# KatiaJDL/CenterPoly

Measured on AMD Instinct MI355X. Metric: inference img/s @2048x1024 DLA-34 (1 GPU), higher is better.
Workload: dtype f32 I/O; split-bf16 x3 contraction (a*b ~ ah*bh + ah*bl + al*bh on bf16 MFMA, ~2^-16 per product) in the convolutions, the heads and DCNv2; f32 accumulate; 1 GPU; BASELINE config 2: DLA-34 + DCNv2, 1x3x1024x2048 synthetic, 16-vertex cartesian head, K=128, forward + sigmoid + NMS/top-k/decode; parallelism=single

## Files before the change

centerpoly_amd/_C.py:

```python
import ctypes
import os
from ctypes import POINTER, Structure, c_char_p, c_float, c_int32, c_int64, c_size_t, c_void_p

import torch

_HERE = os.path.dirname(os.path.abspath(__file__))
LIB_PATH = os.path.join(_HERE, "csrc", "libcenterpoly_hip.so")

CP_OK = 0
REP = {"cartesian": 0, "polar": 1, "polar_fixed": 2}
HEATMAP_UMICH, HEATMAP_ELLIPSE = 0, 1
L1_PLAIN, L1_POLAR, L1_POLAR_FIXED, L1_RELU20, L1_SMOOTH = 0, 1, 2, 3, 4
DCN_BWD_EXACT_F32, DCN_BWD_NARROW_TILES = 1, 2
DCN_CONTRACTION = {"f32": 0, "bf16x3": 1, "bf16x3_region": 3}


class DcnShape(Structure):
    _fields_ = [(n, c_int32) for n in ("B", "Cin", "H", "W", "Cout", "kh", "kw", "stride", "pad",
                                       "dil", "deformable_groups")]


class TargetShape(Structure):
    _fields_ = [(n, c_int32) for n in ("B", "max_objs", "nbr_points", "num_classes", "out_h", "out_w",
                                       "rep", "no_reorder_flip")]
# ... 13 lines not shown
    pass


_lib = None

ABI_VERSION = 3
_P = c_void_p
_SIGNATURES = {
    "cp_abi_version": (c_int32, []),
    "cp_strerror": (c_char_p, [c_int32]),
    "cp_build_arch": (c_char_p, []),
    "cp_dcn_v2_forward_workspace_bytes": (c_size_t, [POINTER(DcnShape)]),
    "cp_dcn_v2_forward_kernel": (c_int32, [POINTER(DcnShape), c_int32]),
    "cp_dcn_v2_forward": (c_int32, [POINTER(DcnShape), _P, _P, c_int64, _P, c_int64, c_int32, _P, _P,
                                    _P, _P, c_int32, c_int32, _P, _P, c_size_t, _P]),
    "cp_dcn_v2_forward_fused_supported": (c_int32, [POINTER(DcnShape)]),
    "cp_dcn_v2_forward_fused_workspace_bytes": (c_size_t, [POINTER(DcnShape)]),
    "cp_dcn_v2_forward_fused": (c_int32, [POINTER(DcnShape), _P, _P, _P, _P, _P, _P, _P, c_int32, c_int32, _P, _P, _P,
                                          c_size_t, _P]),
    "cp_dcn_v2_backward_workspace_bytes": (c_size_t, [POINTER(DcnShape)]),
    "cp_dcn_v2_backward": (c_int32, [POINTER(DcnShape), _P, _P, c_int64, _P, c_int64, c_int32, _P, _P,
                                     _P, _P, c_int64, _P, c_int64, _P, _P, c_int32, _P, c_size_t, _P]),
    "cp_upsample2x_add": (c_int32, [_P, _P, _P] + [c_int32] * 4 + [_P]),
    "cp_depthwise_up_forward": (c_int32, [_P, _P, _P, _P] + [c_int32] * 5 + [_P]),
    "cp_depthwise_up_backward": (c_int32, [_P, _P, _P, _P, _P] + [c_int32] * 5 + [_P]),
    "cp_bn_workspace_bytes": (c_size_t, [c_int32, c_int32, c_int64]),
    "cp_bn_act_forward_train": (c_int32, [_P] * 9 + [c_float, c_float, c_int32, c_int32, c_int32, c_int64,
                                                    _P, c_size_t, _P]),
    "cp_bn_act_backward": (c_int32, [_P] * 7 + [c_int32] + [_P] * 4 + [c_int32, c_int32, c_int64, _P,
                                                                       c_size_t, _P]),
# ... 217 lines not shown
```

centerpoly_amd/csrc/dcn_fwd.hip:

```cpp
#include "cp_common.h"
#include "dcn_internal.h"
#include <stdlib.h>

namespace {

constexpr int BM = 64;
constexpr int TAPS = 9;
#ifndef CP_DCN_LDPAD
#define CP_DCN_LDPAD 2
#endif
constexpr int LDPAD = CP_DCN_LDPAD;
typedef unsigned u32x2 __attribute__((ext_vector_type(2)));
typedef float f32x2 __attribute__((ext_vector_type(2)));

struct DcnFwdArgs {
  const float* x;
  const float* offset;
  const float* mask;
  const float* weight;
  const float* bias;
  const float* ep_scale;
  const float* ep_shift;
  float* out;
  float* partial;
// ... 397 lines not shown
        *reinterpret_cast<f32x4*>(dst) = f32x4{v[0], v[1], v[2], v[3]};
      } else {
#pragma unroll
        for (int r = 0; r < 4; ++r)
          if (pp + r < HWo) dst[r] = v[r];
      }
    }
  }
}

__global__ __launch_bounds__(256) void dcn_splitk_reduce_kernel(DcnFwdArgs a, long long n_per_b) {
  const long long total = (long long)a.B * n_per_b;
  const int HWo = a.Ho * a.Wo;
  for (long long i = (long long)blockIdx.x * 256 + threadIdx.x; i < total;
       i += (long long)gridDim.x * 256) {
    float v = 0.f;
    for (int sidx = 0; sidx < a.splitk; ++sidx) v += a.partial[(long long)sidx * total + i];
    const int co = (int)((i % n_per_b) / HWo);
    float sc = 1.f, sh = 0.f;
    if (a.ep_scale) sc = a.ep_scale[co];
    if (a.ep_shift) sh = a.ep_shift[co];
    else if (a.bias) sh = a.bias[co];
    v = v * sc + sh;
    if (a.relu) v = fmaxf(v, 0.f);
    a.out[i] = v;
  }
}

struct Plan {
  int bn, splitk, c_per_split;
};

Plan make_plan(int B, int Cin, int Cout, int HWo) {
  const long long tiles_m = (long long)((HWo + BM - 1) / BM) * B;
  Plan p;
  p.bn = Cout > 64 ? 128 : 64;
  const long long blocks = tiles_m * ((Cout + p.bn - 1) / p.bn);
  p.splitk = 1;
  const int kc = 4;
  if (blocks < 384) {
    int s = (int)((512 + blocks - 1) / blocks);
// ... 115 lines not shown
  const bool prepared = contraction == CP_DCN_BF16X3_PREPARED || contraction == CP_DCN_BF16X3_REGION_PREPARED;
  const bool bf = contraction == CP_DCN_BF16X3 || contraction == CP_DCN_BF16X3_PREPARED || force_region;
  if (force_region && !cp_dcn_region_supported(s)) return CP_EUNSUPPORTED;
  if (bf && cp_dcn_region_supported(s) && (force_region || region_pays(s))) {
    if (!workspace || workspace_bytes < cp_dcn_v2_forward_workspace_bytes(s)) return CP_EWORKSPACE;
    hipStream_t st = (hipStream_t)stream;
    if (!prepared) {
      const int rc = cp_dcn_region_prepare(s, weight, workspace, st);
      if (rc != CP_OK) return rc;
    }
    const int ks = region_ksplit(s);
    float* partial = ks > 1 ? (float*)((char*)workspace + wpb) : nullptr;
    const int rc = cp_dcn_region_forward(s, x, offset, offset_bstride, mask, mask_bstride, mask_is_logit, workspace, bias,
                                         ep_scale, ep_shift, relu, out, nullptr, nullptr, nullptr, partial, ks, st);
    if (rc != CP_OK || ks <= 1) return rc;
    DcnFwdArgs ra;
    ra.partial = partial; ra.out = out; ra.bias = bias; ra.ep_scale = ep_scale; ra.ep_shift = ep_shift; ra.relu = relu;
    ra.B = s->B; ra.Ho = Ho; ra.Wo = Wo; ra.Cout = s->Cout; ra.splitk = ks;
    const long long n_per_b = (long long)s->Cout * Ho * Wo;
    long long nb = ((long long)s->B * n_per_b + 255) / 256;
    if (nb > 4096) nb = 4096;
    hipLaunchKernelGGL(dcn_splitk_reduce_kernel, dim3((unsigned)nb), dim3(256), 0, st, ra, n_per_b);
    return cp_launch_status();
  }
  if (p.splitk > 1 || bf) {
    if (!workspace || workspace_bytes < cp_dcn_v2_forward_workspace_bytes(s)) return CP_EWORKSPACE;
  }
  DcnFwdArgs a;
  a.x = x; a.offset = offset; a.mask = mask; a.weight = weight; a.bias = bias;
  a.ep_scale = ep_scale; a.ep_shift = ep_shift; a.out = out; a.partial = (float*)((char*)workspace + (workspace ? wpb : 0));
  a.offset_bstride = offset_bstride; a.mask_bstride = mask_bstride;
  a.B = s->B; a.Cin = s->Cin; a.H = s->H; a.W = s->W; a.Cout = s->Cout; a.Ho = Ho; a.Wo = Wo;
  a.stride = s->stride; a.pad = s->pad; a.dil = s->dil;
  a.mask_is_logit = mask_is_logit; a.relu = relu;
  a.splitk = p.splitk; a.c_per_split = p.c_per_split;
#ifdef CP_ABLATE
  {
// ... 4 lines not shown
  hipStream_t st = (hipStream_t)stream;
  CP_CHECK_ARG(contraction == CP_DCN_F32 || bf);
  if ((unsigned long long)s->Cout * s->Cin * 9ull * 4ull >= 0xE0000000ull) return CP_EUNSUPPORTED;
  if (bf && p.bn <= 128 && (p.c_per_split % 8) == 0) {
    if (!prepared) {
      const int nchunk = (s->Cin + 7) / 8;
      const int total = (int)(wperm_bytes_gather(s->Cin, s->Cout) / 16);
      hipLaunchKernelGGL(dcn_fwd_wperm_kernel, dim3((total + 255) / 256), dim3(256), 0, st, weight, (bf16x8*)workspace,
                         s->Cout, s->Cin, nchunk, total);
    }
    if (p.bn == 64) return launch_bf16x3<64, 2>(a, workspace, st);
    return launch_bf16x3<128, 2>(a, workspace, st);
  }
  if (p.bn == 64) return launch_pipe<64, 3>(a, st);
  return launch_pipe<128, 2>(a, st);
}

static size_t fused_region_bytes(const cp_dcn_shape* s) { return cp_align_up(cp_dcn_region_wperm_bytes(s), 256); }

extern "C" int cp_dcn_v2_forward_fused_supported(const cp_dcn_shape* s) {
  return s && s->B > 0 && s->Cout > 0 && s->Cout <= 64 && s->Cin <= 64 && cp_dcn_region_supported(s) && region_pays(s) &&
                 region_ksplit(s) == 1
             ? 1
             : 0;
}

extern "C" size_t cp_dcn_v2_forward_fused_workspace_bytes(const cp_dcn_shape* s) {
  if (!cp_dcn_v2_forward_fused_supported(s)) return 0;
  return fused_region_bytes(s) + cp_align_up(cp_dcn_region_om_wperm_bytes(s), 256);
}
// ... 20 lines not shown
```

centerpoly_amd/csrc/dcn_internal.h:

```cpp
#pragma once
#include "cp_common.h"

static inline int out_extent(int in, int pad, int dil, int stride) {
  return (in + 2 * pad - (dil * 2 + 1)) / stride + 1;
}

bool cp_dcn_region_supported(const cp_dcn_shape* s);
size_t cp_dcn_region_wperm_bytes(const cp_dcn_shape* s);
int cp_dcn_region_prepare(const cp_dcn_shape* s, const float* weight, void* wp, hipStream_t st);
size_t cp_dcn_region_om_wperm_bytes(const cp_dcn_shape* s);
int cp_dcn_region_prepare_om(const cp_dcn_shape* s, const float* om_weight, void* wp, hipStream_t st);
int cp_dcn_region_ksplit(const cp_dcn_shape* s);
int cp_dcn_region_forward(const cp_dcn_shape* s, const float* x, const float* offset, int64_t offset_bstride,
                          const float* mask, int64_t mask_bstride, int32_t mask_is_logit, const void* wp,
                          const float* bias, const float* ep_scale, const float* ep_shift, int32_t relu, float* out,
                          const void* om_wp, const float* om_bias, float* om_out, float* partial, int ksplit,
                          hipStream_t st);

bool cp_dcn_bwd_data2_supported(const cp_dcn_shape* s);
size_t cp_dcn_bwd_data2_workspace_bytes(const cp_dcn_shape* s);
int cp_dcn_bwd_data2(const cp_dcn_shape* s, const float* x, const float* offset, int64_t offset_bstride,
                     const float* mask, int64_t mask_bstride, int32_t mask_is_logit, const float* weight,
                     const float* grad_out, float* grad_x, float* grad_offset, int64_t grad_offset_bstride,
                     float* grad_mask, int64_t grad_mask_bstride, int32_t flags, void* workspace, size_t workspace_bytes,
// ... 7 lines not shown
```

centerpoly_amd/csrc/upsample.hip:

```cpp
#include "cp_common.h"

namespace {

typedef float f32x2 __attribute__((ext_vector_type(2)));

template <int F>
__global__ __launch_bounds__(256) void dw_up_kernel(const float* __restrict__ x,
                                                    const float* __restrict__ w,
                                                    const float* __restrict__ skip,
                                                    float* __restrict__ out, int C, int H, int W) {
  constexpr int KS = 2 * F, PAD = F / 2;
  const int Ho = H * F, Wo = W * F;
  const int bc = blockIdx.z;
  const int c = bc % C;
  const int oy = blockIdx.y;
  const int ox0 = (blockIdx.x * 256 + threadIdx.x) * 4;
  if (ox0 >= Wo) return;
  const float* wc = w + (long long)c * KS * KS;
  const float* xc = x + (long long)bc * H * W;
  const int ky0 = (oy + PAD) % F;
  const int iy0 = (oy + PAD - ky0) / F;
  float v[4] = {0.f, 0.f, 0.f, 0.f};
#pragma unroll
  for (int r = 0; r < 2; ++r) {
// ... 14 lines not shown
  }
  const long long o = ((long long)bc * Ho + oy) * Wo + ox0;
  if (skip) {
    if (ox0 + 3 < Wo) {
      const f32x4 s = *reinterpret_cast<const f32x4*>(skip + o);
      v[0] += s[0]; v[1] += s[1]; v[2] += s[2]; v[3] += s[3];
    } else {
      for (int q = 0; q < 4 && ox0 + q < Wo; ++q) v[q] += skip[o + q];
    }
  }
  if (ox0 + 3 < Wo) *reinterpret_cast<f32x4*>(out + o) = f32x4{v[0], v[1], v[2], v[3]};
  else
    for (int q = 0; q < 4 && ox0 + q < Wo; ++q) out[o + q] = v[q];
}

__global__ __launch_bounds__(256) void dw_up2_kernel(const float* __restrict__ x, const float* __restrict__ w,
                                                     const float* __restrict__ skip, float* __restrict__ out, int C, int H,
                                                     int W) {
  const int W2 = W >> 1;
  const int bc = blockIdx.y;
  const int idx = blockIdx.x * 256 + threadIdx.x;
  if (idx >= H * W2) return;
  const int i = idx / W2, j = idx - i * W2;
  const float* wc = w + (long long)(bc % C) * 16;
  float wk[4][4];
#pragma unroll
  for (int a = 0; a < 4; ++a)
#pragma unroll
    for (int b = 0; b < 4; ++b) wk[a][b] = wc[a * 4 + b];
  const float* xc = x + (long long)bc * H * W;
  float in[3][4];
#pragma unroll
  for (int r = 0; r < 3; ++r) {
    const int iy = i - 1 + r;
    const bool rok = iy >= 0 && iy < H;
    const float* row = xc + (long long)(rok ? iy : i) * W + 2 * j;
    const f32x2 mid = *reinterpret_cast<const f32x2*>(row);
    const float lft = j > 0 ? row[-1] : 0.f, rgt = 2 * j + 2 < W ? row[2] : 0.f;
    in[r][0] = rok ? lft : 0.f;
    in[r][1] = rok ? mid[0] : 0.f;
    in[r][2] = rok ? mid[1] : 0.f;
    in[r][3] = rok ? rgt : 0.f;
  }
  const int Wo = 2 * W;
  const long long o = ((long long)bc * 2 * H + 2 * i) * Wo + 4 * j;
#pragma unroll
  for (int e = 0; e < 2; ++e) {
    const float* hi = in[1 + e];
    const float* lo = in[e];
    const float* wa = wk[1 - e];
    const float* wb = wk[3 - e];
    f32x4 v;
    v[0] = hi[1] * wa[1] + hi[0] * wa[3] + lo[1] * wb[1] + lo[0] * wb[3];
    v[1] = hi[2] * wa[0] + hi[1] * wa[2] + lo[2] * wb[0] + lo[1] * wb[2];
    v[2] = hi[2] * wa[1] + hi[1] * wa[3] + lo[2] * wb[1] + lo[1] * wb[3];
    v[3] = hi[3] * wa[0] + hi[2] * wa[2] + lo[3] * wb[0] + lo[2] * wb[2];
    if (skip) {
      const f32x4 sk = *reinterpret_cast<const f32x4*>(skip + o + (long long)e * Wo);
      v[0] += sk[0]; v[1] += sk[1]; v[2] += sk[2]; v[3] += sk[3];
    }
    *reinterpret_cast<f32x4*>(out + o + (long long)e * Wo) = v;
  }
}

}

extern "C" int cp_depthwise_up_forward(const float* x, const float* weight, const float* skip,
                                       float* out, int32_t B, int32_t C, int32_t H, int32_t W,
                                       int32_t f, void* stream) {
  CP_CHECK_ARG(x && weight && out && B > 0 && C > 0 && H > 0 && W > 0);
  if (f != 2 && f != 4 && f != 8) return CP_EUNSUPPORTED;
  if ((W * f) % 4 != 0 || (long long)B * C > 65535 || (long long)H * f > 65535) return CP_EUNSUPPORTED;
  const int Wo = W * f, Ho = H * f;
  dim3 grid((Wo / 4 + 255) / 256, Ho, B * C);
  hipStream_t st = (hipStream_t)stream;
  if (f == 2 && (W & 1) == 0 && (long long)H * (W / 2) < (1ll << 31) - 256) {
    const dim3 g2((unsigned)(((long long)H * (W / 2) + 255) / 256), B * C);
    hipLaunchKernelGGL(dw_up2_kernel, g2, dim3(256), 0, st, x, weight, skip, out, C, H, W);
  } else if (f == 2) hipLaunchKernelGGL(dw_up_kernel<2>, grid, dim3(256), 0, st, x, weight, skip, out, C, H, W);
  else if (f == 4) hipLaunchKernelGGL(dw_up_kernel<4>, grid, dim3(256), 0, st, x, weight, skip, out, C, H, W);
  else hipLaunchKernelGGL(dw_up_kernel<8>, grid, dim3(256), 0, st, x, weight, skip, out, C, H, W);
  return cp_launch_status();
}

namespace {
__global__ __launch_bounds__(256) void bias_act_kernel(float* __restrict__ y,
                                                       const float* __restrict__ bias,
                                                       const float* __restrict__ res, int C,
                                                       long long HW, int relu) {
  const int bc = blockIdx.y;
  const float bv = bias ? bias[bc % C] : 0.f;
  float* yp = y + (long long)bc * HW;
  const float* rp = res ? res + (long long)bc * HW : nullptr;
  const long long n4 = HW >> 2;
  for (long long i = (long long)blockIdx.x * 256 + threadIdx.x; i < n4; i += (long long)gridDim.x * 256) {
    f32x4 v = reinterpret_cast<f32x4*>(yp)[i];
// ... 379 lines not shown
```

centerpoly_amd/models/networks/DCNv2/dcn_v2.py:

```python
import math
import os

import torch
import torch.nn.functional as F
import torch.nn as nn
from torch.nn.modules.utils import _pair

from .... import _C
from ..conv3x3 import conv_bias_act, conv_infer, conv_raw
from ..prepared import prepared


def _shape(x, weight, stride, pad, dil, dg):
    s = _C.DcnShape()
    s.B, s.Cin, s.H, s.W = x.shape
    s.Cout, _, s.kh, s.kw = weight.shape
    s.stride, s.pad, s.dil, s.deformable_groups = stride, pad, dil, dg
    return s


_AUTO = {}


def auto_contraction(s):
# ... 25 lines not shown
        if not built:
            mode += 1
    elif nws:
        ws = _C.workspace(nws, x.device)
    timer = _C.kernel_timer
    end = timer.start(("dcn_fwd", s.Cin, s.Cout, Ho, Wo, s.B)) if timer is not None else None
    rc = L.cp_dcn_v2_forward(s, _C.ptr(x), _C.ptr(om), bs, mask_ptr, bs, 1, _C.ptr(weight),
                             _C.ptr(bias), _C.ptr(ep_scale), _C.ptr(ep_shift), 1 if relu else 0,
                             mode, _C.ptr(out), _C.ptr(ws), nws, _C.stream())
    if end is not None:
        end.record()
    _C.check(rc, "cp_dcn_v2_forward")
    return out


def dcn_v2_module_forward(x, om_weight, om_bias, weight, bias, ep_scale=None, ep_shift=None, relu=False, owner=None,
                          want_om=False):
    L = _C.lib()
    s = _shape(x, weight, 1, 1, 1, 1)
    if tuple(weight.shape[2:]) != (3, 3) or tuple(om_weight.shape) != (27, s.Cin, 3, 3) \
            or not L.cp_dcn_v2_forward_fused_supported(s):
        return None
    nws = L.cp_dcn_v2_forward_fused_workspace_bytes(s)
    ws, built = (_C.workspace(nws, x.device), True) if owner is None else \
        prepared(owner, "dcn_fused", (weight, om_weight), lambda: _C.workspace(nws, x.device), tuple(x.shape))
    out = torch.empty((s.B, s.Cout, s.H, s.W), dtype=torch.float32, device=x.device)
    om = torch.empty((s.B, 27, s.H, s.W), dtype=torch.float32, device=x.device) if want_om else None
    timer = _C.kernel_timer
    end = timer.start(("dcn_fwd", s.Cin, s.Cout, s.H, s.W, s.B)) if timer is not None else None
    rc = L.cp_dcn_v2_forward_fused(s, _C.ptr(x), _C.ptr(om_weight), _C.ptr(om_bias), _C.ptr(weight), _C.ptr(bias),
# ... 174 lines not shown
    def forward_fused(self, x, ep_scale, ep_shift, relu=True):
        cm = self.conv_offset_mask
        con = getattr(self, "contraction", None) or DCN.infer_contraction
        if DCN.fuse_offset_conv and con in ("auto", "bf16x3") and x.is_cuda and x.dtype == torch.float32 \
                and self.stride == 1 and self.padding == 1 and self.dilation == 1 and self.deformable_groups == 1:
            r = dcn_v2_module_forward(x.contiguous(), cm.weight, cm.bias, self.weight, None, ep_scale, ep_shift, relu,
                                      owner=self)
            if r is not None:
                return r[0]
        om = conv_infer([x], cm, cm.weight, cm.bias, conv=cm)
        if om is None:
            om = cm(x)
        return dcn_v2_forward_raw(x.contiguous(), om.contiguous(), self.weight, None, self.stride,
                                  self.padding, self.dilation, self.deformable_groups, ep_scale,
                                  ep_shift, relu, getattr(self, "contraction", None) or DCN.infer_contraction, owner=self)
```

centerpoly_amd/models/networks/pose_dla_dcn.py:

```python
import math
import os

import numpy as np
import torch
import torch.nn.functional as F
from torch import nn

from ... import _C
from .DCNv2.dcn_v2 import DCN, conv_bias
from . import conv3x3
from .conv3x3 import conv_infer, conv_raw
from .prepared import prepared, release_inference

HEADS_FUSED = True
CONV_DIRECT_WGRAD = True

BN_MOMENTUM = 0.1


def _bn(c):
    return nn.BatchNorm2d(c, momentum=BN_MOMENTUM)



# ... 358 lines not shown
                              root_dim=root_dim + out_channels, **kw)
        self.downsample = nn.MaxPool2d(stride, stride=stride) if stride > 1 else None
        self.project = None
        if in_channels != out_channels:
            self.project = nn.Sequential(nn.Conv2d(in_channels, out_channels, 1, 1, bias=False),
                                         _bn(out_channels))
        self.project_is_dead = levels > 1 and self.project is not None
        if self.project_is_dead:
            for prm in self.project.parameters():
                prm.requires_grad_(False)

    def fold(self):
        self._folded = _fold_conv_bn(self.project[0], self.project[1]) if self.project is not None \
            else None

    def forward(self, x, residual=None, children=None):
        children = [] if children is None else children
        bottom = x if self.downsample is None else downsample2(self.downsample, x)
        if self.project is None:
            residual = bottom
        elif self.project_is_dead:
            residual = None
            if self.training:
                with torch.no_grad():
                    if bottom.is_cuda:
                        bn_act(self.project[1], conv_train(self.project[0], bottom), relu=False)
                    else:
                        self.project(bottom)
        elif _use_folded(self):
            residual = _conv_folded(bottom, self.project[0], self._folded)
        else:
            residual = bn_act(self.project[1], conv_train(self.project[0], bottom), relu=False)
        if self.level_root:
            children.append(bottom)
        x1 = self.tree1(x, residual)
        if self.levels == 1:
            return self.root(self.tree2(x1), x1, *children)
        children.append(x1)
        return self.tree2(x1, children=children)


class DLA(nn.Module):
    def __init__(self, levels, channels, num_classes=1000, block=BasicBlock, residual_root=False,
                 linear_root=False):
        super().__init__()
        self.channels, self.num_classes = channels, num_classes
        c = channels
        self.base_layer = nn.Sequential(nn.Conv2d(3, c[0], 7, 1, 3, bias=False), _bn(c[0]),
                                        nn.ReLU(inplace=True))
        self.level0 = self._conv_level(c[0], c[0], levels[0])
# ... 90 lines not shown
        return scale.contiguous(), shift.contiguous()

    def fold(self):
        with torch.no_grad():
            self._folded = self.folded_affine()

    def forward(self, x):
        if not self.training and not torch.is_grad_enabled():
            scale, shift = self._folded if getattr(self, "_folded", None) is not None \
                else self.folded_affine()
            return self.conv.forward_fused(x, scale, shift, relu=True)
        if self.training:
            return bn_act(self.actf[0], self.conv(x), relu=True)
        return self.actf(self.conv(x))


def depthwise_up_add(x, up, skip):
    L = _C.lib()
    B, C, H, W = x.shape
    f = up.stride[0]
    out = torch.empty((B, C, H * f, W * f), dtype=torch.float32, device=x.device)
    x, skip = x.contiguous(), skip.contiguous()
    rc = L.cp_depthwise_up_forward(_C.ptr(x), _C.ptr(up.weight), _C.ptr(skip), _C.ptr(out), B, C, H,
                                   W, f, _C.stream())
    _C.check(rc, "cp_depthwise_up_forward")
    return out


class _DepthwiseUpAdd(torch.autograd.Function):

# ... 13 lines not shown
    @staticmethod
    def backward(ctx, go):
        x, weight = ctx.saved_tensors
        L = _C.lib()
        go = go.contiguous()
        B, C, H, W = x.shape
        gx = torch.empty_like(x)
        gw = _C.zeros(weight.shape, weight.device)
        rc = L.cp_depthwise_up_backward(_C.ptr(x), _C.ptr(weight), _C.ptr(go), _C.ptr(gx), _C.ptr(gw),
                                        B, C, H, W, ctx.f, _C.stream())
        _C.check(rc, "cp_depthwise_up_backward")
        return gx, gw, go, None


class IDAUp(nn.Module):
    def __init__(self, o, channels, up_f):
        super().__init__()
        for i in range(1, len(channels)):
            f = int(up_f[i])
            up = nn.ConvTranspose2d(o, o, f * 2, stride=f, padding=f // 2, output_padding=0,
                                    groups=o, bias=False)
            fill_up_weights(up)
            setattr(self, "proj_%d" % i, DeformConv(channels[i], o))
            setattr(self, "up_%d" % i, up)
            setattr(self, "node_%d" % i, DeformConv(o, o))

    def forward(self, layers, startp, endp):
        fused = not self.training and not torch.is_grad_enabled()
        for i in range(startp + 1, endp):
            k = i - startp
            up, proj = getattr(self, "up_%d" % k), getattr(self, "proj_%d" % k)
            aligned = layers[i].is_cuda and (layers[i].shape[3] * up.stride[0]) % 4 == 0
            if fused and aligned and up.stride[0] in (2, 4, 8):
                summed = depthwise_up_add(proj(layers[i]), up, layers[i - 1])
            elif not fused and aligned and up.stride[0] in (2, 4):
                summed = _DepthwiseUpAdd.apply(proj(layers[i]), up.weight, layers[i - 1], up.stride[0])
            else:
                summed = up(proj(layers[i])) + layers[i - 1]
            layers[i] = getattr(self, "node_%d" % k)(summed)


class DLAUp(nn.Module):
    def __init__(self, startp, channels, scales, in_channels=None):
        super().__init__()
        self.startp = startp
        in_channels = list(channels) if in_channels is None else in_channels
        self.channels = channels
        channels = list(channels)
        scales = np.array(scales, dtype=int)
# ... 188 lines not shown
```

include/centerpoly_hip.h:

```cpp
#ifndef CENTERPOLY_HIP_H
#define CENTERPOLY_HIP_H

#include <stddef.h>
#include <stdint.h>

#ifdef __cplusplus
extern "C" {
#endif

#define CP_ABI_VERSION 3

enum {
  CP_OK = 0,
  CP_EINVAL = -1,
  CP_EUNSUPPORTED = -2,
  CP_EWORKSPACE = -3,
  CP_EHIP = -4
};

enum { CP_REP_CARTESIAN = 0, CP_REP_POLAR = 1, CP_REP_POLAR_FIXED = 2 };

enum {
  CP_DCN_F32 = 0,
  CP_DCN_BF16X3 = 1,
// ... 16 lines not shown

typedef struct cp_dcn_shape {
  int32_t B, Cin, H, W, Cout;
  int32_t kh, kw, stride, pad, dil;
  int32_t deformable_groups;
} cp_dcn_shape;

size_t cp_dcn_v2_forward_workspace_bytes(const cp_dcn_shape* s);
int cp_dcn_v2_forward_kernel(const cp_dcn_shape* s, int32_t contraction);
int cp_dcn_v2_forward(const cp_dcn_shape* s, const float* x, const float* offset,
                      int64_t offset_bstride, const float* mask, int64_t mask_bstride,
                      int32_t mask_is_logit, const float* weight, const float* bias,
                      const float* ep_scale, const float* ep_shift, int32_t relu,
                      int32_t contraction, float* out, void* workspace, size_t workspace_bytes,
                      void* stream);

int cp_dcn_v2_forward_fused_supported(const cp_dcn_shape* s);
size_t cp_dcn_v2_forward_fused_workspace_bytes(const cp_dcn_shape* s);
int cp_dcn_v2_forward_fused(const cp_dcn_shape* s, const float* x, const float* om_weight, const float* om_bias,
                            const float* weight, const float* bias, const float* ep_scale, const float* ep_shift,
                            int32_t relu, int32_t prepared, float* om_out, float* out, void* workspace,
                            size_t workspace_bytes, void* stream);

enum {
  CP_DCN_BWD_EXACT_F32 = 1,
  CP_DCN_BWD_NARROW_TILES = 2
};
size_t cp_dcn_v2_backward_workspace_bytes(const cp_dcn_shape* s);
int cp_dcn_v2_backward(const cp_dcn_shape* s, const float* x, const float* offset,
                       int64_t offset_bstride, const float* mask, int64_t mask_bstride,
                       int32_t mask_is_logit, const float* weight, const float* grad_out,
                       float* grad_x, float* grad_offset, int64_t grad_offset_bstride,
                       float* grad_mask, int64_t grad_mask_bstride, float* grad_weight,
                       float* grad_bias, int32_t flags, void* workspace, size_t workspace_bytes, void* stream);

int cp_depthwise_up_forward(const float* x, const float* weight, const float* skip, float* out,
                            int32_t B, int32_t C, int32_t H, int32_t W, int32_t f, void* stream);
int cp_depthwise_up_backward(const float* x, const float* weight, const float* grad_out,
                             float* grad_x, float* grad_weight, int32_t B, int32_t C, int32_t H,
                             int32_t W, int32_t f, void* stream);

int cp_maxpool2x2_forward(const float* x, float* out, int32_t B, int32_t C, int32_t H, int32_t W, void* stream);
int cp_maxpool2x2_backward(const float* x, const float* grad_out, float* grad_in, int32_t B, int32_t C, int32_t H,
                           int32_t W, void* stream);

int cp_upsample2x_add(const float* a, const float* low, float* out, int32_t B, int32_t C, int32_t H, int32_t W,
                      void* stream);

int cp_bias_act_inplace(float* y, const float* bias, const float* residual, int32_t B, int32_t C,
                        int64_t HW, int32_t relu, void* stream);
int cp_bias_relu_backward(const float* y, const float* grad_out, float* grad_in, float* grad_bias,
                          int32_t B, int32_t C, int64_t HW, void* stream);
// ... 259 lines not shown
```

Measured before the change: 358.1 img/s.

## Fold DCN split-K reduction into depthwise upsample-add and share Tree pooling

In IDAUp, the DCN projection now leaves its split-K partial slices in the workspace. A new tiled depthwise-upsample kernel sums those slices, applies the folded BN affine and ReLU in shared memory, then performs the 2x transposed depthwise upsample plus skip add. This removes the separate split-K reduce kernel and one full round trip of the projection output through memory. It also adds a dedicated 4x upsample kernel, an unrolled slice-summing helper, and reuse of the downsampled tensor between a Tree and its tree1 child at inference, so the same maxpool is not computed twice.

```diff
diff --git a/centerpoly_amd/_C.py b/centerpoly_amd/_C.py
--- a/centerpoly_amd/_C.py
+++ b/centerpoly_amd/_C.py
@@ -51,6 +51,11 @@
     "cp_dcn_v2_forward_kernel": (c_int32, [POINTER(DcnShape), c_int32]),
     "cp_dcn_v2_forward": (c_int32, [POINTER(DcnShape), _P, _P, c_int64, _P, c_int64, c_int32, _P, _P,
                                     _P, _P, c_int32, c_int32, _P, _P, c_size_t, _P]),
+    "cp_dcn_v2_forward_slices_count": (c_int32, [POINTER(DcnShape), c_int32]),
+    "cp_dcn_v2_forward_slices": (c_int32, [POINTER(DcnShape), _P, _P, c_int64, _P, c_int64, c_int32, _P, c_int32, _P,
+                                           c_size_t, POINTER(c_size_t), _P]),
+    "cp_dcn_splitk_reduce": (c_int32, [_P, c_int32, _P, _P, c_int32, _P, c_int32, c_int32, c_int64, _P]),
+    "cp_depthwise_up_forward_slices": (c_int32, [_P, c_int32, c_int64, _P, _P, c_int32, _P, _P, _P] + [c_int32] * 5 + [_P]),
     "cp_dcn_v2_forward_fused_supported": (c_int32, [POINTER(DcnShape)]),
     "cp_dcn_v2_forward_fused_workspace_bytes": (c_size_t, [POINTER(DcnShape)]),
     "cp_dcn_v2_forward_fused": (c_int32, [POINTER(DcnShape), _P, _P, _P, _P, _P, _P, _P, c_int32, c_int32, _P, _P, _P,
diff --git a/centerpoly_amd/csrc/dcn_fwd.hip b/centerpoly_amd/csrc/dcn_fwd.hip
--- a/centerpoly_amd/csrc/dcn_fwd.hip
+++ b/centerpoly_amd/csrc/dcn_fwd.hip
@@ -435,17 +435,27 @@
   const int HWo = a.Ho * a.Wo;
   for (long long i = (long long)blockIdx.x * 256 + threadIdx.x; i < total;
        i += (long long)gridDim.x * 256) {
-    float v = 0.f;
-    for (int sidx = 0; sidx < a.splitk; ++sidx) v += a.partial[(long long)sidx * total + i];
     const int co = (int)((i % n_per_b) / HWo);
     float sc = 1.f, sh = 0.f;
     if (a.ep_scale) sc = a.ep_scale[co];
     if (a.ep_shift) sh = a.ep_shift[co];
     else if (a.bias) sh = a.bias[co];
-    v = v * sc + sh;
-    if (a.relu) v = fmaxf(v, 0.f);
-    a.out[i] = v;
-  }
+    const float* p[1] = {a.partial + i};
+    float v[1];
+    cp_dcn_slices_values<1>(p, total, a.splitk, sc, sh, a.relu, v);
+    a.out[i] = v[0];
+  }
+}
+
+void launch_splitk_reduce(const float* partial, int ks, const float* bias, const float* ep_scale, const float* ep_shift,
+                          int relu, float* out, int B, int Cout, int Ho, int Wo, hipStream_t st) {
+  DcnFwdArgs ra;
+  ra.partial = const_cast<float*>(partial); ra.out = out; ra.bias = bias; ra.ep_scale = ep_scale; ra.ep_shift = ep_shift;
+  ra.relu = relu; ra.B = B; ra.Ho = Ho; ra.Wo = Wo; ra.Cout = Cout; ra.splitk = ks;
+  const long long n_per_b = (long long)Cout * Ho * Wo;
+  long long nb = ((long long)B * n_per_b + 255) / 256;
+  if (nb > 4096) nb = 4096;
+  hipLaunchKernelGGL(dcn_splitk_reduce_kernel, dim3((unsigned)nb), dim3(256), 0, st, ra, n_per_b);
 }
 
 struct Plan {
@@ -591,13 +601,7 @@
     const int rc = cp_dcn_region_forward(s, x, offset, offset_bstride, mask, mask_bstride, mask_is_logit, workspace, bias,
                                          ep_scale, ep_shift, relu, out, nullptr, nullptr, nullptr, partial, ks, st);
     if (rc != CP_OK || ks <= 1) return rc;
-    DcnFwdArgs ra;
-    ra.partial = partial; ra.out = out; ra.bias = bias; ra.ep_scale = ep_scale; ra.ep_shift = ep_shift; ra.relu = relu;
-    ra.B = s->B; ra.Ho = Ho; ra.Wo = Wo; ra.Cout = s->Cout; ra.splitk = ks;
-    const long long n_per_b = (long long)s->Cout * Ho * Wo;
-    long long nb = ((long long)s->B * n_per_b + 255) / 256;
-    if (nb > 4096) nb = 4096;
-    hipLaunchKernelGGL(dcn_splitk_reduce_kernel, dim3((unsigned)nb), dim3(256), 0, st, ra, n_per_b);
+    launch_splitk_reduce(partial, ks, bias, ep_scale, ep_shift, relu, out, s->B, s->Cout, Ho, Wo, st);
     return cp_launch_status();
   }
   if (p.splitk > 1 || bf) {
@@ -632,6 +636,47 @@
   }
   if (p.bn == 64) return launch_pipe<64, 3>(a, st);
   return launch_pipe<128, 2>(a, st);
+}
+
+extern "C" int cp_dcn_v2_forward_slices_count(const cp_dcn_shape* s, int32_t contraction) {
+  if (!s || s->B <= 0 || s->Cin <= 0 || s->H <= 0 || s->W < 2 || s->Cout <= 0) return 0;
+  if (s->kh != 3 || s->kw != 3 || s->deformable_groups != 1 || s->stride <= 0 || s->dil <= 0 || s->pad < 0) return 0;
+  const bool force = contraction == CP_DCN_BF16X3_REGION || contraction == CP_DCN_BF16X3_REGION_PREPARED;
+  if (contraction != CP_DCN_BF16X3 && contraction != CP_DCN_BF16X3_PREPARED && !force) return 0;
+  if (!cp_dcn_region_supported(s) || !(force || region_pays(s))) return 0;
+  if ((long long)s->H * s->W >= (1ll << 31)) return 0;
+  const Plan p = make_plan(s->B, s->Cin, s->Cout, s->H * s->W);
+  if ((long long)s->B * p.splitk > 65535) return 0;
+  const int ks = region_ksplit(s);
+  return ks > 1 ? ks : 0;
+}
+
+extern "C" int cp_dcn_v2_forward_slices(const cp_dcn_shape* s, const float* x, const float* offset, int64_t offset_bstride,
+                                        const float* mask, int64_t mask_bstride, int32_t mask_is_logit,
+                                        const float* weight, int32_t contraction, void* workspace, size_t workspace_bytes,
+                                        size_t* partial_offset, void* stream) {
+  CP_CHECK_ARG(s && x && offset && mask && weight && partial_offset);
+  const int ks = cp_dcn_v2_forward_slices_count(s, contraction);
+  if (ks <= 1) return CP_EUNSUPPORTED;
+  if (!workspace || workspace_bytes < cp_dcn_v2_forward_workspace_bytes(s)) return CP_EWORKSPACE;
+  hipStream_t st = (hipStream_t)stream;
+  const bool prepared = contraction == CP_DCN_BF16X3_PREPARED || contraction == CP_DCN_BF16X3_REGION_PREPARED;
+  if (!prepared) {
+    const int rc = cp_dcn_region_prepare(s, weight, workspace, st);
+    if (rc != CP_OK) return rc;
+  }
+  const size_t wpb = wperm_bytes(s);
+  *partial_offset = wpb;
+  return cp_dcn_region_forward(s, x, offset, offset_bstride, mask, mask_bstride, mask_is_logit, workspace, nullptr, nullptr,
+                               nullptr, 0, nullptr, nullptr, nullptr, nullptr, (float*)((char*)workspace + wpb), ks, st);
+}
+
+extern "C" int cp_dcn_splitk_reduce(const float* partial, int32_t nslices, const float* ep_scale, const float* ep_shift,
+                                    int32_t relu, float* out, int32_t B, int32_t C, int64_t HW, void* stream) {
+  CP_CHECK_ARG(partial && out && nslices > 0 && B > 0 && C > 0 && HW > 0);
+  if (HW >= (1ll << 31)) return CP_EUNSUPPORTED;
+  launch_splitk_reduce(partial, nslices, nullptr, ep_scale, ep_shift, relu, out, B, C, 1, (int)HW, (hipStream_t)stream);
+  return cp_launch_status();
 }
 
 static size_t fused_region_bytes(const cp_dcn_shape* s) { return cp_align_up(cp_dcn_region_wperm_bytes(s), 256); }
diff --git a/centerpoly_amd/csrc/dcn_internal.h b/centerpoly_amd/csrc/dcn_internal.h
--- a/centerpoly_amd/csrc/dcn_internal.h
+++ b/centerpoly_amd/csrc/dcn_internal.h
@@ -3,6 +3,41 @@
 
 static inline int out_extent(int in, int pad, int dil, int stride) {
   return (in + 2 * pad - (dil * 2 + 1)) / stride + 1;
+}
+
+template <int N, int U>
+__device__ __forceinline__ void cp_dcn_slices_block(const float* (&p)[N], long long stride, int sidx, float (&v)[N]) {
+  float t[U][N];
+#pragma unroll
+  for (int u = 0; u < U; ++u)
+#pragma unroll
+    for (int k = 0; k < N; ++k) t[u][k] = p[k][(long long)(sidx + u) * stride];
+#pragma unroll
+  for (int u = 0; u < U; ++u)
+#pragma unroll
+    for (int k = 0; k < N; ++k) v[k] += t[u][k];
+}
+
+template <int N>
+__device__ inline void cp_dcn_slices_values(const float* (&p)[N], long long stride, int nslices, float sc, float sh,
+                                            int relu, float (&v)[N]) {
+#pragma unroll
+  for (int k = 0; k < N; ++k) v[k] = 0.f;
+  int sidx = 0;
+  for (; sidx + 8 <= nslices; sidx += 8) cp_dcn_slices_block<N, 8>(p, stride, sidx, v);
+  if (sidx + 4 <= nslices) {
+    cp_dcn_slices_block<N, 4>(p, stride, sidx, v);
+    sidx += 4;
+  }
+  for (; sidx < nslices; ++sidx) {
+#pragma unroll
+    for (int k = 0; k < N; ++k) v[k] += p[k][(long long)sidx * stride];
+  }
+#pragma unroll
+  for (int k = 0; k < N; ++k) {
+    v[k] = v[k] * sc + sh;
+    if (relu) v[k] = fmaxf(v[k], 0.f);
+  }
 }
 
 bool cp_dcn_region_supported(const cp_dcn_shape* s);
diff --git a/centerpoly_amd/csrc/upsample.hip b/centerpoly_amd/csrc/upsample.hip
--- a/centerpoly_amd/csrc/upsample.hip
+++ b/centerpoly_amd/csrc/upsample.hip
@@ -1,4 +1,5 @@
 #include "cp_common.h"
+#include "dcn_internal.h"
 
 namespace {
 
@@ -52,6 +53,68 @@
     for (int q = 0; q < 4 && ox0 + q < Wo; ++q) out[o + q] = v[q];
 }
 
+template <int R>
+__device__ __forceinline__ void load_skip_rows(const float* __restrict__ skip, long long o, int Wo, f32x4 (&sk)[R]) {
+#pragma unroll
+  for (int e = 0; e < R; ++e)
+    sk[e] = skip ? *reinterpret_cast<const f32x4*>(skip + o + (long long)e * Wo) : f32x4{0.f, 0.f, 0.f, 0.f};
+}
+
+__device__ __forceinline__ void up2_patch_store(const float (&in)[3][4], const float* __restrict__ wc,
+                                                const f32x4 (&sk)[2], bool has_skip, float* __restrict__ out, long long o,
+                                                int Wo) {
+  float wk[4][4];
+#pragma unroll
+  for (int a = 0; a < 4; ++a)
+#pragma unroll
+    for (int b = 0; b < 4; ++b) wk[a][b] = wc[a * 4 + b];
+#pragma unroll
+  for (int e = 0; e < 2; ++e) {
+    const float* hi = in[1 + e];
+    const float* lo = in[e];
+    const float* wa = wk[1 - e];
+    const float* wb = wk[3 - e];
+    f32x4 v;
+    v[0] = hi[1] * wa[1] + hi[0] * wa[3] + lo[1] * wb[1] + lo[0] * wb[3];
+    v[1] = hi[2] * wa[0] + hi[1] * wa[2] + lo[2] * wb[0] + lo[1] * wb[2];
+    v[2] = hi[2] * wa[1] + hi[1] * wa[3] + lo[2] * wb[1] + lo[1] * wb[3];
+    v[3] = hi[3] * wa[0] + hi[2] * wa[2] + lo[3] * wb[0] + lo[2] * wb[2];
+    if (has_skip) {
+      v[0] += sk[e][0]; v[1] += sk[e][1]; v[2] += sk[e][2]; v[3] += sk[e][3];
+    }
+    *reinterpret_cast<f32x4*>(out + o + (long long)e * Wo) = v;
+  }
+}
+
+__device__ __forceinline__ void up4_patch_store(const float (&in)[3][3], const float* __restrict__ wc,
+                                                const f32x4 (&sk)[4], bool has_skip, float* __restrict__ out, long long o,
+                                                int Wo) {
+  float wk[8][8];
+#pragma unroll
+  for (int a = 0; a < 8; ++a)
+#pragma unroll
+    for (int b = 0; b < 8; ++b) wk[a][b] = wc[a * 8 + b];
+#pragma unroll
+  for (int e = 0; e < 4; ++e) {
+    const int rh = e < 2 ? 1 : 2, kyh = e < 2 ? 2 + e : e - 2;
+    f32x4 v;
+#pragma unroll
+    for (int q = 0; q < 4; ++q) {
+      const int ch = q < 2 ? 1 : 2, kxh = q < 2 ? 2 + q : q - 2;
+      float s = 0.f;
+      s += in[rh][ch] * wk[kyh][kxh];
+      s += in[rh][ch - 1] * wk[kyh][kxh + 4];
+      s += in[rh - 1][ch] * wk[kyh + 4][kxh];
+      s += in[rh - 1][ch - 1] * wk[kyh + 4][kxh + 4];
+      v[q] = s;
+    }
+    if (has_skip) {
+      v[0] += sk[e][0]; v[1] += sk[e][1]; v[2] += sk[e][2]; v[3] += sk[e][3];
+    }
+    *reinterpret_cast<f32x4*>(out + o + (long long)e * Wo) = v;
+  }
+}
+
 __global__ __launch_bounds__(256) void dw_up2_kernel(const float* __restrict__ x, const float* __restrict__ w,
                                                      const float* __restrict__ skip, float* __restrict__ out, int C, int H,
                                                      int W) {
@@ -61,11 +124,6 @@
   if (idx >= H * W2) return;
   const int i = idx / W2, j = idx - i * W2;
   const float* wc = w + (long long)(bc % C) * 16;
-  float wk[4][4];
-#pragma unroll
-  for (int a = 0; a < 4; ++a)
-#pragma unroll
-    for (int b = 0; b < 4; ++b) wk[a][b] = wc[a * 4 + b];
   const float* xc = x + (long long)bc * H * W;
   float in[3][4];
 #pragma unroll
@@ -80,24 +138,92 @@
     in[r][2] = rok ? mid[1] : 0.f;
     in[r][3] = rok ? rgt : 0.f;
   }
-  const int Wo = 2 * W;
-  const long long o = ((long long)bc * 2 * H + 2 * i) * Wo + 4 * j;
-#pragma unroll
-  for (int e = 0; e < 2; ++e) {
-    const float* hi = in[1 + e];
-    const float* lo = in[e];
-    const float* wa = wk[1 - e];
-    const float* wb = wk[3 - e];
-    f32x4 v;
-    v[0] = hi[1] * wa[1] + hi[0] * wa[3] + lo[1] * wb[1] + lo[0] * wb[3];
-    v[1] = hi[2] * wa[0] + hi[1] * wa[2] + lo[2] * wb[0] + lo[1] * wb[2];
-    v[2] = hi[2] * wa[1] + hi[1] * wa[3] + lo[2] * wb[1] + lo[1] * wb[3];
-    v[3] = hi[3] * wa[0] + hi[2] * wa[2] + lo[3] * wb[0] + lo[2] * wb[2];
-    if (skip) {
-      const f32x4 sk = *reinterpret_cast<const f32x4*>(skip + o + (long long)e * Wo);
-      v[0] += sk[0]; v[1] += sk[1]; v[2] += sk[2]; v[3] += sk[3];
-    }
-    *reinterpret_cast<f32x4*>(out + o + (long long)e * Wo) = v;
+  const long long o = ((long long)bc * 2 * H + 2 * i) * (2 * W) + 4 * j;
+  f32x4 sk[2];
+  load_skip_rows<2>(skip, o, 2 * W, sk);
+  up2_patch_store(in, wc, sk, skip != nullptr, out, o, 2 * W);
+}
+
+__global__ __launch_bounds__(256) void dw_up4_kernel(const float* __restrict__ x, const float* __restrict__ w,
+                                                     const float* __restrict__ skip, float* __restrict__ out, int C, int H,
+                                                     int W) {
+  const int bc = blockIdx.y;
+  const int idx = blockIdx.x * 256 + threadIdx.x;
+  if (idx >= H * W) return;
+  const int i = idx / W, j = idx - i * W;
+  const float* xc = x + (long long)bc * H * W;
+  float in[3][3];
+#pragma unroll
+  for (int r = 0; r < 3; ++r) {
+    const int iy = i - 1 + r;
+    const bool rok = iy >= 0 && iy < H;
+    const float* row = xc + (long long)(rok ? iy : i) * W + j;
+    const float lft = j > 0 ? row[-1] : 0.f, mid = row[0], rgt = j + 1 < W ? row[1] : 0.f;
+    in[r][0] = rok ? lft : 0.f;
+    in[r][1] = rok ? mid : 0.f;
+    in[r][2] = rok ? rgt : 0.f;
+  }
+  const long long o = ((long long)bc * 4 * H + 4 * i) * (4 * W) + 4 * j;
+  f32x4 sk[4];
+  load_skip_rows<4>(skip, o, 4 * W, sk);
+  up4_patch_store(in, w + (long long)(bc % C) * 64, sk, skip != nullptr, out, o, 4 * W);
+}
+
+template <int F>
+__global__ __launch_bounds__(256) void dw_up_slices_kernel(const float* __restrict__ partial, int nslices,
+                                                           long long slice_stride, const float* __restrict__ ep_scale,
+                                                           const float* __restrict__ ep_shift, int relu,
+                                                           const float* __restrict__ w, const float* __restrict__ skip,
+                                                           float* __restrict__ out, int C, int H, int W, int tiles_x) {
+  constexpr int PW = F == 2 ? 2 : 1;
+  constexpr int TH = 8, TW = 32 * PW;
+  __shared__ float tile[TH + 2][TW + 2];
+  const int bc = blockIdx.y, c = bc % C;
+  const int ty = blockIdx.x / tiles_x;
+  const int y0 = ty * TH, x0 = (blockIdx.x - ty * tiles_x) * TW;
+  const float sc = ep_scale ? ep_scale[c] : 1.f, sh = ep_shift ? ep_shift[c] : 0.f;
+  const float* pc = partial + (long long)bc * H * W;
+  const int li = threadIdx.x >> 5, lj = (threadIdx.x & 31) * PW;
+  const int i = y0 + li, jx = x0 + lj;
+  const bool live = i < H && jx < W;
+  const int Wo = F * W;
+  const long long o = ((long long)bc * F * H + F * i) * Wo + F * jx;
+  f32x4 sk[F];
+  load_skip_rows<F>(live ? skip : nullptr, o, Wo, sk);
+  constexpr int TOTAL = (TH + 2) * (TW + 2), NE = (TOTAL + 255) / 256;
+  const float* p[NE];
+  bool inside[NE];
+  int slot[NE];
+#pragma unroll
+  for (int k = 0; k < NE; ++k) {
+    const int e = min((int)threadIdx.x + 256 * k, TOTAL - 1);
+    const int r = e / (TW + 2), q = e - r * (TW + 2);
+    const int iy = y0 - 1 + r, ix = x0 - 1 + q;
+    inside[k] = iy >= 0 && iy < H && ix >= 0 && ix < W;
+    slot[k] = (int)threadIdx.x + 256 * k < TOTAL ? e : -1;
+    p[k] = pc + (long long)min(max(iy, 0), H - 1) * W + min(max(ix, 0), W - 1);
+  }
+  float v[NE];
+  cp_dcn_slices_values<NE>(p, slice_stride, nslices, sc, sh, relu, v);
+#pragma unroll
+  for (int k = 0; k < NE; ++k)
+    if (slot[k] >= 0) (&tile[0][0])[slot[k]] = inside[k] ? v[k] : 0.f;
+  __syncthreads();
+  if (!live) return;
+  if constexpr (F == 2) {
+    float in[3][4];
+#pragma unroll
+    for (int r = 0; r < 3; ++r)
+#pragma unroll
+      for (int k = 0; k < 4; ++k) in[r][k] = tile[li + r][lj + k];
+    up2_patch_store(in, w + (long long)c * 16, sk, skip != nullptr, out, o, Wo);
+  } else {
+    float in[3][3];
+#pragma unroll
+    for (int r = 0; r < 3; ++r)
+#pragma unroll
+      for (int k = 0; k < 3; ++k) in[r][k] = tile[li + r][lj + k];
+    up4_patch_store(in, w + (long long)c * 64, sk, skip != nullptr, out, o, Wo);
   }
 }
 
@@ -116,8 +242,33 @@
     const dim3 g2((unsigned)(((long long)H * (W / 2) + 255) / 256), B * C);
     hipLaunchKernelGGL(dw_up2_kernel, g2, dim3(256), 0, st, x, weight, skip, out, C, H, W);
   } else if (f == 2) hipLaunchKernelGGL(dw_up_kernel<2>, grid, dim3(256), 0, st, x, weight, skip, out, C, H, W);
-  else if (f == 4) hipLaunchKernelGGL(dw_up_kernel<4>, grid, dim3(256), 0, st, x, weight, skip, out, C, H, W);
+  else if (f == 4 && (long long)H * W < (1ll << 31) - 256) {
+    const dim3 g4((unsigned)(((long long)H * W + 255) / 256), B * C);
+    hipLaunchKernelGGL(dw_up4_kernel, g4, dim3(256), 0, st, x, weight, skip, out, C, H, W);
+  } else if (f == 4) hipLaunchKernelGGL(dw_up_kernel<4>, grid, dim3(256), 0, st, x, weight, skip, out, C, H, W);
   else hipLaunchKernelGGL(dw_up_kernel<8>, grid, dim3(256), 0, st, x, weight, skip, out, C, H, W);
+  return cp_launch_status();
+}
+
+extern "C" int cp_depthwise_up_forward_slices(const float* partial, int32_t nslices, int64_t slice_stride,
+                                              const float* ep_scale, const float* ep_shift, int32_t relu,
+                                              const float* weight, const float* skip, float* out, int32_t B, int32_t C,
+                                              int32_t H, int32_t W, int32_t f, void* stream) {
+  CP_CHECK_ARG(partial && weight && out && nslices > 0 && slice_stride >= 0 && B > 0 && C > 0 && H > 0 && W > 0);
+  if (!((f == 2 && (W & 1) == 0) || f == 4)) return CP_EUNSUPPORTED;
+  if ((long long)B * C > 65535) return CP_EUNSUPPORTED;
+  const int tw = f == 2 ? 64 : 32;
+  const int tiles_x = (W + tw - 1) / tw;
+  const long long tiles = (long long)tiles_x * ((H + 7) / 8);
+  if (tiles >= (1ll << 31)) return CP_EUNSUPPORTED;
+  const dim3 grid((unsigned)tiles, B * C);
+  hipStream_t st = (hipStream_t)stream;
+  if (f == 2)
+    hipLaunchKernelGGL(dw_up_slices_kernel<2>, grid, dim3(256), 0, st, partial, nslices, (long long)slice_stride, ep_scale,
+                       ep_shift, relu, weight, skip, out, C, H, W, tiles_x);
+  else
+    hipLaunchKernelGGL(dw_up_slices_kernel<4>, grid, dim3(256), 0, st, partial, nslices, (long long)slice_stride, ep_scale,
+                       ep_shift, relu, weight, skip, out, C, H, W, tiles_x);
   return cp_launch_status();
 }
 
diff --git a/centerpoly_amd/models/networks/DCNv2/dcn_v2.py b/centerpoly_amd/models/networks/DCNv2/dcn_v2.py
--- a/centerpoly_amd/models/networks/DCNv2/dcn_v2.py
+++ b/centerpoly_amd/models/networks/DCNv2/dcn_v2.py
@@ -63,6 +63,43 @@
     return out
 
 
+def dcn_v2_slices_count(x, weight, stride=1, pad=1, dil=1, dg=1, contraction="f32"):
+    s = _shape(x, weight, stride, pad, dil, dg)
+    if contraction == "auto":
+        contraction = auto_contraction(s)
+    return _C.lib().cp_dcn_v2_forward_slices_count(s, _C.DCN_CONTRACTION[contraction])
+
+
+def dcn_v2_forward_slices(x, om, weight, stride=1, pad=1, dil=1, dg=1, contraction="f32", owner=None):
+    L = _C.lib()
+    s = _shape(x, weight, stride, pad, dil, dg)
+    Ho, Wo = om.shape[2], om.shape[3]
+    K = s.kh * s.kw
+    bs = 3 * K * Ho * Wo
+    mask_ptr = _C.c_void_p(om.data_ptr() + 4 * 2 * K * Ho * Wo)
+    nws = L.cp_dcn_v2_forward_workspace_bytes(s)
+    if contraction == "auto":
+        contraction = auto_contraction(s)
+    mode = _C.DCN_CONTRACTION[contraction]
+    nsl = L.cp_dcn_v2_forward_slices_count(s, mode)
+    if owner is not None and mode in (1, 3):
+        ws, built = prepared(owner, "dcn_fwd", (weight,), lambda: _C.workspace(nws, x.device),
+                             (mode, tuple(x.shape), tuple(om.shape)))
+        if not built:
+            mode += 1
+    else:
+        ws = _C.workspace(nws, x.device)
+    off = _C.c_size_t(0)
+    timer = _C.kernel_timer
+    end = timer.start(("dcn_fwd", s.Cin, s.Cout, Ho, Wo, s.B)) if timer is not None else None
+    rc = L.cp_dcn_v2_forward_slices(s, _C.ptr(x), _C.ptr(om), bs, mask_ptr, bs, 1, _C.ptr(weight), mode, _C.ptr(ws), nws,
+                                    _C.ctypes.byref(off), _C.stream())
+    if end is not None:
+        end.record()
+    _C.check(rc, "cp_dcn_v2_forward_slices")
+    return ws, off.value, nsl
+
+
 def dcn_v2_module_forward(x, om_weight, om_bias, weight, bias, ep_scale=None, ep_shift=None, relu=False, owner=None,
                           want_om=False):
     L = _C.lib()
@@ -267,3 +304,17 @@
         return dcn_v2_forward_raw(x.contiguous(), om.contiguous(), self.weight, None, self.stride,
                                   self.padding, self.dilation, self.deformable_groups, ep_scale,
                                   ep_shift, relu, getattr(self, "contraction", None) or DCN.infer_contraction, owner=self)
+
+    def forward_slices(self, x):
+        if not (x.is_cuda and x.dtype == torch.float32):
+            return None
+        con = getattr(self, "contraction", None) or DCN.infer_contraction
+        x = x.contiguous()
+        cfg = (self.stride, self.padding, self.dilation, self.deformable_groups)
+        if dcn_v2_slices_count(x, self.weight, *cfg, contraction=con) <= 1:
+            return None
+        cm = self.conv_offset_mask
+        om = conv_infer([x], cm, cm.weight, cm.bias, conv=cm)
+        if om is None:
+            om = cm(x)
+        return dcn_v2_forward_slices(x, om.contiguous(), self.weight, *cfg, contraction=con, owner=self)
diff --git a/centerpoly_amd/models/networks/pose_dla_dcn.py b/centerpoly_amd/models/networks/pose_dla_dcn.py
--- a/centerpoly_amd/models/networks/pose_dla_dcn.py
+++ b/centerpoly_amd/models/networks/pose_dla_dcn.py
@@ -396,9 +396,18 @@
         self._folded = _fold_conv_bn(self.project[0], self.project[1]) if self.project is not None \
             else None
 
-    def forward(self, x, residual=None, children=None):
+    share_pool = True
+
+    def _same_pool(self, other):
+        a, b = self.downsample, getattr(other, "downsample", None)
+        return isinstance(other, Tree) and a is not None and b is not None and \
+            (a.kernel_size, a.stride, a.padding, a.dilation, a.ceil_mode) == \
+            (b.kernel_size, b.stride, b.padding, b.dilation, b.ceil_mode)
+
+    def forward(self, x, residual=None, children=None, bottom=None):
         children = [] if children is None else children
-        bottom = x if self.downsample is None else downsample2(self.downsample, x)
+        if bottom is None:
+            bottom = x if self.downsample is None else downsample2(self.downsample, x)
         if self.project is None:
             residual = bottom
         elif self.project_is_dead:
@@ -415,7 +424,10 @@
             residual = bn_act(self.project[1], conv_train(self.project[0], bottom), relu=False)
         if self.level_root:
             children.append(bottom)
-        x1 = self.tree1(x, residual)
+        if Tree.share_pool and self.levels > 1 and not torch.is_grad_enabled() and self._same_pool(self.tree1):
+            x1 = self.tree1(x, residual, bottom=bottom)
+        else:
+            x1 = self.tree1(x, residual)
         if self.levels == 1:
             return self.root(self.tree2(x1), x1, *children)
         children.append(x1)
@@ -536,6 +548,32 @@
             return bn_act(self.actf[0], self.conv(x), relu=True)
         return self.actf(self.conv(x))
 
+    def forward_slices(self, x):
+        r = self.conv.forward_slices(x)
+        if r is None:
+            return None
+        scale, shift = self._folded if getattr(self, "_folded", None) is not None else self.folded_affine()
+        return r + (scale, shift)
+
+
+def depthwise_up_add_slices(proj, x, up, skip):
+    f = up.stride[0]
+    B, _, H, W = x.shape
+    C = up.weight.shape[0]
+    if f not in IDAUp.fold_slices_factors or (f == 2 and W % 2) or B * C > 65535:
+        return None
+    r = proj.forward_slices(x)
+    if r is None:
+        return None
+    ws, off, nsl, scale, shift = r
+    out = torch.empty((B, C, H * f, W * f), dtype=torch.float32, device=x.device)
+    skip = skip.contiguous()
+    rc = _C.lib().cp_depthwise_up_forward_slices(_C.c_void_p(ws.data_ptr() + off), nsl, B * C * H * W, _C.ptr(scale),
+                                                 _C.ptr(shift), 1, _C.ptr(up.weight), _C.ptr(skip), _C.ptr(out), B, C, H,
+                                                 W, f, _C.stream())
+    _C.check(rc, "cp_depthwise_up_forward_slices")
+    return out
+
 
 def depthwise_up_add(x, up, skip):
     L = _C.lib()
@@ -579,6 +617,9 @@
 
 
 class IDAUp(nn.Module):
+    fold_slices = True
+    fold_slices_factors = (2,)
+
     def __init__(self, o, channels, up_f):
         super().__init__()
         for i in range(1, len(channels)):
@@ -597,7 +638,9 @@
             up, proj = getattr(self, "up_%d" % k), getattr(self, "proj_%d" % k)
             aligned = layers[i].is_cuda and (layers[i].shape[3] * up.stride[0]) % 4 == 0
             if fused and aligned and up.stride[0] in (2, 4, 8):
-                summed = depthwise_up_add(proj(layers[i]), up, layers[i - 1])
+                summed = depthwise_up_add_slices(proj, layers[i], up, layers[i - 1]) if IDAUp.fold_slices else None
+                if summed is None:
+                    summed = depthwise_up_add(proj(layers[i]), up, layers[i - 1])
             elif not fused and aligned and up.stride[0] in (2, 4):
                 summed = _DepthwiseUpAdd.apply(proj(layers[i]), up.weight, layers[i - 1], up.stride[0])
             else:
diff --git a/include/centerpoly_hip.h b/include/centerpoly_hip.h
--- a/include/centerpoly_hip.h
+++ b/include/centerpoly_hip.h
@@ -54,6 +54,14 @@
                       const float* ep_scale, const float* ep_shift, int32_t relu,
                       int32_t contraction, float* out, void* workspace, size_t workspace_bytes,
                       void* stream);
+
+int cp_dcn_v2_forward_slices_count(const cp_dcn_shape* s, int32_t contraction);
+int cp_dcn_v2_forward_slices(const cp_dcn_shape* s, const float* x, const float* offset, int64_t offset_bstride,
+                             const float* mask, int64_t mask_bstride, int32_t mask_is_logit, const float* weight,
+                             int32_t contraction, void* workspace, size_t workspace_bytes, size_t* partial_offset,
+                             void* stream);
+int cp_dcn_splitk_reduce(const float* partial, int32_t nslices, const float* ep_scale, const float* ep_shift,
+                         int32_t relu, float* out, int32_t B, int32_t C, int64_t HW, void* stream);
 
 int cp_dcn_v2_forward_fused_supported(const cp_dcn_shape* s);
 size_t cp_dcn_v2_forward_fused_workspace_bytes(const cp_dcn_shape* s);
@@ -76,6 +84,9 @@
 
 int cp_depthwise_up_forward(const float* x, const float* weight, const float* skip, float* out,
                             int32_t B, int32_t C, int32_t H, int32_t W, int32_t f, void* stream);
+int cp_depthwise_up_forward_slices(const float* partial, int32_t nslices, int64_t slice_stride, const float* ep_scale,
+                                   const float* ep_shift, int32_t relu, const float* weight, const float* skip,
+                                   float* out, int32_t B, int32_t C, int32_t H, int32_t W, int32_t f, void* stream);
 int cp_depthwise_up_backward(const float* x, const float* weight, const float* grad_out,
                              float* grad_x, float* grad_weight, int32_t B, int32_t C, int32_t H,
                              int32_t W, int32_t f, void* stream);
```

Result: faster. 367.9 img/s (median of 6 runs) (+2.7%).
